# HSarham/automatic-ar

Measured on AMD Instinct MI355X. Metric: LM iterations/sec, higher is better.
Workload: dtype f64

## Files before the change

### automatic-ar_amd/csrc/ba_capi.hip

```cpp
#include <hip/hip_runtime.h>
#include <dlfcn.h>
#include <execinfo.h>
#include <fcntl.h>
#include <unistd.h>
#include <signal.h>

#include <algorithm>
#include <array>
#include <atomic>
#include <chrono>
#include <cmath>
#include <cstring>
#include <map>
#include <numeric>
#include <condition_variable>
#include <mutex>
#include <vector>

#include "../host/internal.h"
#include "../host/se3.h"
#include "geom.hpp"
#include "hostcopy.h"
#include "kernels.h"

// ... 1446 lines not shown
        P.Ad = ((int)dense_ent.size() + 31) / 32 * 32;
        dense_ent.resize(P.Ad, -1);
        const int nga = P.Ad / 16, ngb = P.Ad / 32;
        std::vector<std::vector<uint8_t>> pa(nga, std::vector<uint8_t>(F, 0)), pb(ngb, std::vector<uint8_t>(F, 0));
        for (int f = 0; f < F; f++) {
            pa[0][f] = pb[0][f] = 1;
            for (int s = fslot_start[f]; s < fslot_start[f + 1]; s++) {
                const int dd = dense_of[fslot_ent[s]];
                pa[dd / 16][f] = 1;
                pb[dd / 32][f] = 1;
            }
        }
        struct Blk { int ga, gb; std::vector<int32_t> fr; };
        std::vector<Blk> blks;
        int64_t total_steps = 0;
        for (int ga = 0; ga < nga; ga++)
            for (int gb = 0; gb <= (16 * ga + 15) / 32; gb++) {
                Blk bk{ga, gb, {}};
                for (int f = 0; f < F; f++)
                    if (pa[ga][f] && pb[gb][f]) bk.fr.push_back(f);
                if (bk.fr.empty()) continue;
                total_steps += ((int64_t)bk.fr.size() + 1) / 2;
                blks.push_back(std::move(bk));
            }
        int target = 12 * (int)blks.size();
        if (const char *e = getenv("AAR_SCHUR_SPLIT")) target = std::max(1, atoi(e)) * (int)blks.size();
        const int64_t plen = std::max<int64_t>(16, ((2 * total_steps + target - 1) / target + 3) / 4 * 4);
        struct Piece { int blk; int64_t b, e; int f0; };
        std::vector<Piece> pieces;
        for (size_t k = 0; k < blks.size(); k++)
            for (int64_t b0 = 0; b0 < (int64_t)blks[k].fr.size(); b0 += plen)
                pieces.push_back({(int)k, b0, std::min<int64_t>(b0 + plen, (int64_t)blks[k].fr.size()), blks[k].fr[b0]});
        std::stable_sort(pieces.begin(), pieces.end(), [](const Piece &x, const Piece &y) { return x.f0 < y.f0; });
        for (const Piece &pc : pieces) {
            sm_ga.push_back(blks[pc.blk].ga); sm_gb.push_back(blks[pc.blk].gb);
            sm_fb.push_back((int32_t)sm_frames.size());
            sm_frames.insert(sm_frames.end(), blks[pc.blk].fr.begin() + pc.b, blks[pc.blk].fr.begin() + pc.e);
            sm_fe.push_back((int32_t)sm_frames.size());
        }
        slot_frame.resize(P.total_slots);
        slot_dense.resize(P.total_slots);
        for (int f = 0; f < F; f++)
            for (int s = fslot_start[f]; s < fslot_start[f + 1]; s++) {
                slot_frame[s] = f;
                slot_dense[s] = dense_of[fslot_ent[s]];
            }
        P.n_smwork = (int)sm_ga.size();
    }

    std::vector<int32_t> ent_fixed(A, 0);
    for (int c = 0; c < C; c++) ent_fixed[c] = (c == L.rc || !L.oc) ? 1 : 0;
    for (int m = 0; m < M; m++) ent_fixed[C + m] = (m == L.rm || !L.om) ? 1 : 0;
    for (int e = 0; e < C + M; e++) ent_fixed[e] |= held[e];
    std::vector<double> Kh(d->cam_mats, d->cam_mats + 9 * (size_t)C);

#define UP(field, vec) if ((rc = dev_upload(pb, &P.field, vec))) return fail(rc)
    UP(K, Kh); UP(a_idx, a_idx); UP(a_uv, a_uv); UP(frame_obs_start, frame_obs_start); UP(frame_stride, frame_stride);
    UP(fslot_start, fslot_start); UP(fslot_ent, fslot_ent); UP(b_idx, b_idx); UP(b_uv, b_uv);
    UP(chunk_start, chunk_start); UP(ent_fixed, ent_fixed); UP(up_start, up_start); UP(up_ent, up_ent);
    UP(sw_ent, sw_ent); UP(sw_begin, sw_begin); UP(sw_end, sw_end); UP(pair_rec, pair_rec);
    if (P.use_pcg) {
        const int cus = P.n_cus;
        int64_t longest = 0;
        for (int a = 0; a < A; a++) longest = std::max<int64_t>(longest, pair_base[a + 1] - pair_base[a]);
        int64_t chunk = std::max<int64_t>(256, (total_pairs + 2LL * cus - 1) / (2LL * cus));
        chunk = std::max<int64_t>(chunk, (longest + 7) / 8);
        if (const char *t = getenv("AAR_PCG_CHUNK")) chunk = std::max<int64_t>((longest + 7) / 8, atoll(t));
        std::vector<int32_t> it_ent, it_begin, it_end, ent_item_start(A + 1, 0);
        for (int a = 0; a < A; a++) {
            ent_item_start[a] = (int32_t)it_ent.size();
            const int64_t b0 = pair_base[a], e0 = ent_fixed[a] ? pair_base[a] : pair_base[a + 1];
            int64_t b = b0;
            do {
                const int64_t e = std::min<int64_t>(e0, b + chunk);
                it_ent.push_back(a); it_begin.push_back((int32_t)b); it_end.push_back((int32_t)e);
                b = e;
            } while (b < e0);
        }
        ent_item_start[A] = (int32_t)it_ent.size();
        P.pcg_n_items = (int)it_ent.size();
        UP(pcg_it_ent, it_ent); UP(pcg_it_begin, it_begin); UP(pcg_it_end, it_end); UP(pcg_ent_item_start, ent_item_start);
    }
    if (P.deterministic) { UP(sp_off, sp_off); UP(se_start, se_start); UP(se_items, se_items); UP(pbr_start, pbr_start); UP(pbr_chunk, pbr_chunk); UP(pbr_kind, pbr_kind); UP(pbr_a, pbr_a); UP(pbr_b, pbr_b); }
    if (P.n_smwork) { UP(sm_ga, sm_ga); UP(sm_gb, sm_gb); UP(sm_fb, sm_fb); UP(sm_fe, sm_fe); UP(slot_dense, slot_dense); UP(slot_frame, slot_frame); UP(dense_ent, dense_ent); UP(sm_frames, sm_frames); }
#undef UP
#define AL(field, count) if ((rc = dev_alloc(pb, &P.field, (size_t)(count)))) return fail(rc)
    AL(z[0], 6 * (size_t)(A + F)); AL(z[1], 6 * (size_t)(A + F));
    AL(ent[0], (size_t)(A + F) * ENT_STRIDE); AL(ent[1], (size_t)(A + F) * ENT_STRIDE);
    for (int w = 0; w < 2; w++) {
        AL(blk[w].V, (size_t)F * 36); AL(blk[w].gf, (size_t)F * 6); AL(blk[w].W, (size_t)P.total_slots * 36);
        AL(blk[w].Vinv, (size_t)F * 36); AL(blk[w].hf, (size_t)F * 6);
        AL(blk[w].S, (size_t)P.n_pad * P.n_pad + 2 * (size_t)P.n_pad + 8);
        P.blk[w].rhs = P.blk[w].S + (size_t)P.n_pad * P.n_pad;
        P.blk[w].g0 = P.blk[w].rhs + P.n_pad;
        P.blk[w].tail = P.blk[w].g0 + P.n_pad;
        if (hipMemset(P.blk[w].tail, 0, 8 * sizeof(double)) != hipSuccess) return fail(set_error(AAR_ERR_HIP, "hipMemset failed"));
    }
    if (P.deterministic) { AL(sp_part, (size_t)sp_total); AL(pb_part, (size_t)P.n_chunks * P.pb_stride); }
    if (P.use_pcg) {
        AL(pcg_ws, (size_t)P.pcg_n_items * 28 + 6 * (size_t)F + 8); AL(pcg_counter, 8);
        AL(pcg_yg, (size_t)3 * PCG_NYV * P.n_pad + (size_t)28 * A + 160 + 8); AL(pcg_hop, 2 * PCG_HOP_WORDS);
        if (const char *t = getenv("AAR_PCG_FUSED")) P.pcg_fused = atoi(t) != 0 ? 1 : 0;
        {
            int w32 = 1;
            if (const char *t = getenv("AAR_PCG_W32")) w32 = atoi(t) != 0 ? 1 : 0;
            if (w32 && P.pcg_fused && !P.deterministic && P.pcg_eta >= PCG_W32_MIN_ETA)
// ... 2037 lines not shown
```

### automatic-ar_amd/csrc/kernels.h

```cpp
#pragma once
#include <hip/hip_runtime.h>
#include <stdint.h>
#include <utility>

namespace aar {

constexpr int CHOL_NB = 96;
constexpr int PASSB_CHUNK = 1024;
constexpr int SPCG_MAX_IT = 128, SPCG_BUFS = SPCG_MAX_IT + 2, SPCG_MAX_NT = 14;
inline int spcg_default_cap(int nT) { return nT <= 4 ? 64 : SPCG_MAX_IT; }
constexpr int PCG_NY = 16;
constexpr int PCG_NYV = 2;
constexpr int PCG_HOP_WORDS = (2 * PCG_NY + 1) * 16;
constexpr double PCG_W32_MIN_ETA = 1e-4;
constexpr double SPCG_ABS_TOL_DEFAULT = 2e-5, PCG_ABS_TOL_DEFAULT = 5e-5;
constexpr double SPCG_ETA_DEFAULT = 3e-4, SPCG_ETA_LOOSE_DEFAULT = 0.0, PCG_ETA_DEFAULT = 5e-3, PCG_ETA_LOOSE_DEFAULT = 0.0;
inline int spcg_stride(int n_pad) { return 8 * (n_pad / 6); }


#ifndef SPCG_PRE
#define SPCG_PRE 0
#endif

enum KernelId { KID_UNPACK = 0, KID_RESIDUAL, KID_PASSA, KID_PASSB, KID_MAXDIAG, KID_FRAME_INV, KID_SCHUR, KID_LDL_DIAG,
                KID_LDL_TRSM, KID_LDL_UPDATE, KID_LDL_BACKSOLVE, KID_BACKSUB, KID_REDUCE, KID_LDL_PANEL, KID_PCG, KID_SPCG, KID_SPCG_PRE, KID_PRIOR, KID_COUNT };

struct LaunchHook {
    void (*pre)(void *ctx, int kid) = nullptr;
    void (*post)(void *ctx, int kid) = nullptr;
    void *ctx = nullptr;
};

struct ObsIdx {
    int32_t frame, cam, marker, slots;
};

struct DeviceProblem {
    int C = 0, M = 0, A = 0;
    int intr = 0;
    int F = 0;
    int64_t N = 0;
    int n = 0, n_pad = 0, nT = 0;
    int total_slots = 0, max_kf = 0;
    int n_chunks = 0, n_swork = 0;
    int res_f32 = 1;
    float huber = -1.f;
    double half_size = 0;
    double *K = nullptr;
    ObsIdx *a_idx = nullptr;
    float *a_uv = nullptr;
    int32_t *frame_obs_start = nullptr;
    int32_t *frame_stride = nullptr;
    int32_t *fslot_start = nullptr;
    int32_t *fslot_ent = nullptr;
    ObsIdx *b_idx = nullptr;
    float *b_uv = nullptr;
    int32_t *chunk_start = nullptr;
    int32_t *ent_fixed = nullptr;
    int frames_fixed = 0;
    int32_t *sw_ent = nullptr, *sw_begin = nullptr, *sw_end = nullptr;
    int4 *pair_rec = nullptr;
    int n_smwork = 0;
    int32_t *sm_ga = nullptr, *sm_gb = nullptr, *sm_fb = nullptr, *sm_fe = nullptr, *sm_frames = nullptr;
    int Ad = 0;
    int32_t *slot_dense = nullptr;
    int32_t *slot_frame = nullptr;
    int32_t *dense_ent = nullptr;
    double *Wd = nullptr, *Yd = nullptr;
    int dense_from_passA = 1;
    int deterministic = 0;
    double *pb_part = nullptr;
    int pb_stride = 0, n_pbr = 0;
    int32_t *pbr_start = nullptr, *pbr_chunk = nullptr, *pbr_kind = nullptr, *pbr_a = nullptr, *pbr_b = nullptr;
    double *sp_part = nullptr;
    int64_t *sp_off = nullptr;
    int32_t *se_start = nullptr, *se_items = nullptr;
    int use_pcg = 0, pcg_grid = 0, pcg_max_it = 200;
    double pcg_eta = 0.1;
    double pcg_eta_loose = 0.0, pcg_eta_switch = 0.01, pcg_eta_now = 0.1;
    double pcg_abs_tol = SPCG_ABS_TOL_DEFAULT;
    int pcg_n_items = 0;
    int32_t *pcg_it_ent = nullptr, *pcg_it_begin = nullptr, *pcg_it_end = nullptr, *pcg_ent_item_start = nullptr;
    double *pcg_ws = nullptr;
    int32_t *pcg_counter = nullptr;
    mutable int pcg_parity = 0;
    int n_cus = 256;
    mutable int want_w64 = 0;
    int pcg_fused = 1;
    int pcg_rank0 = 1;
    int pcg_resident = 1;
    int pcg_e_every = 1;
    mutable int pcg_e_age = 0;
    int pcg_coarse = 1, pcg_coarse_from = 8;
    int32_t *up_start = nullptr, *up_ent = nullptr;
    double *pcg_yg = nullptr;
    int32_t *pcg_hop = nullptr;
    int use_spcg = 0, spcg_max_it = 64;
    int spcg_spread = 8;
    int spcg_coarse = 1;
    int spcg_coarse_from = 12;
    mutable int spcg_coarse_on = 0;
    double *spcg_pre = nullptr;
    mutable int spcg_pre_epoch = 0;
    int spcg_root_c = -1, spcg_root_m = -1, spcg_n_free = 0;
    int spcg_test_drop = -1;
    double *spcg_ws = nullptr;
    int32_t *spcg_iters = nullptr;
    mutable int spcg_parity = 0;
    int32_t *spcg_done = nullptr;
    mutable int spcg_epoch = 0;
    double *pcgd_setup = nullptr, *pcgd_minv = nullptr, *pcgd_state = nullptr, *pcgd_y = nullptr, *pcgd_host = nullptr;
    struct Tuning {
        int fused_panel = 3;
        int bs_rides = 1;
        int backsub_rides = 0;
        int lookahead = 1;
        int passA_variant = 0;
        int passAB_occ2 = -1;
        int spcg_backsub_rides = 0;
        int passA_wrench = 1;
        int passB_wrench_merged = 0;
        int passB_lean = 0;
        int pack_system = -1;
        int init_headstart = 1;
    } tune;
    double *z[2] = {nullptr, nullptr};
    double *ent[2] = {nullptr, nullptr};
    struct Blocks {
        double *V = nullptr, *gf = nullptr;
        double *W = nullptr;
        float *Wf = nullptr;
        double *Vinv = nullptr, *hf = nullptr;
        double *S = nullptr;
        double *rhs = nullptr;
        double *g0 = nullptr;
        double *tail = nullptr;
    } blk[2];
    double *Dfac = nullptr;
    double *Linv16 = nullptr;
    double *Lp = nullptr;
    double *zf = nullptr;
    double *delta_s = nullptr;
    int32_t *bs_flags = nullptr;
    mutable int bs_epoch = 0;
    double *err_part = nullptr;
    double *lin_part = nullptr;
    double *scal = nullptr;
    double *host_result = nullptr;
    int32_t *flags = nullptr;
    double *r_out = nullptr;
    int n_prior = 0, prior_rank0 = 1;
    int32_t *prior_ent = nullptr;
    double *prior_dat = nullptr;
    double *prior_out = nullptr;
    LaunchHook hook;
};

void raise_dynamic_lds(const void *kernel, size_t bytes);
template <typename... Params, typename... Args>
inline void launch_lds(void (*kernel)(Params...), dim3 grid, dim3 block, size_t lds, hipStream_t st, Args &&...args) {
    raise_dynamic_lds(reinterpret_cast<const void *>(kernel), lds);
    hipLaunchKernelGGL(kernel, grid, block, lds, st, std::forward<Args>(args)...);
}

struct KTable { const double *base; int stride; };
constexpr int ENT_STRIDE_H = 24;
inline KTable k_table(const DeviceProblem &P, int which) {
    if (P.intr) return KTable{P.ent[which] + (size_t)(P.C + P.M) * ENT_STRIDE_H, ENT_STRIDE_H};
    return KTable{P.K, 9};
}
constexpr int SLOT_C_BITS = 10, SLOT_M_BITS = 11;
inline int pack_slots(int sc, int sm, int sk) { return sc | (sm << SLOT_C_BITS) | (sk << (SLOT_C_BITS + SLOT_M_BITS)); }

extern volatile int g_last_kernel_id;
struct HookScope {
    const DeviceProblem &P;
    int kid;
    HookScope(const DeviceProblem &p, int k) : P(p), kid(k) { g_last_kernel_id = k; if (P.hook.pre) P.hook.pre(P.hook.ctx, kid); }
    ~HookScope() { if (P.hook.post) P.hook.post(P.hook.ctx, kid); }
};

void launch_unpack(const DeviceProblem &P, int which, hipStream_t st, int zero_blk = -1);
void launch_residual(const DeviceProblem &P, int which, double *r_out, hipStream_t st);
void launch_passA(const DeviceProblem &P, int which, double mu_pred, int zero_blk, hipStream_t st);
void launch_passB(const DeviceProblem &P, int which, hipStream_t st);
bool launch_passAB(const DeviceProblem &P, int which, double mu_pred, int zero_blk, hipStream_t st);
size_t passA_lds_bytes(int max_kf, int block);
size_t passA_wrench_lds_bytes(int max_kf, bool intr);
void launch_maxdiag(const DeviceProblem &P, int which, hipStream_t st);
void launch_frame_inv(const DeviceProblem &P, int which, double mu, hipStream_t st, const double *mu_dev = nullptr, double mu_scale = 0.0);
bool launch_schur(const DeviceProblem &P, int which, double sign, hipStream_t st, unsigned long long ride_seq = 0, int ride_n_err = 0,
                  double *ride_scal = nullptr, bool panels_ready = false);
bool launch_chol(const DeviceProblem &P, int which, double mu, hipStream_t st, int trial = -1);
void launch_backsub(const DeviceProblem &P, int cur, int trial, hipStream_t st);
void launch_pcg(const DeviceProblem &P, int which, double mu, hipStream_t st);
size_t pcg_lds_bytes(int A, bool coarse = false);
int pcg_max_grid(int A, bool coarse, int cus);
bool launch_spcg(const DeviceProblem &P, int which, double mu, hipStream_t st, int trial = -1);
int spcg_resident_per_cu(int nT, bool coarse);
inline bool spcg_coarse_now(const DeviceProblem &P) { return P.spcg_coarse && (P.spcg_root_c >= 0 || P.spcg_root_m >= 0); }
bool spcg_fits(int nT);
size_t spcg_ws_doubles(int n_pad);
size_t spcg_pre_doubles(int n_pad);
void spcg_ws_reset(const DeviceProblem &P, hipStream_t st);
void launch_pcgd_setup(const DeviceProblem &P, int which, double mu, hipStream_t st);
void launch_pcgd_iter(const DeviceProblem &P, int which, double mu, int k, bool last, unsigned long long publish_seq, hipStream_t st);
double *pcgd_y_of_launch(const DeviceProblem &P, int k);
void launch_reduce_scalars(const DeviceProblem &P, int n_err, bool fold_shared, unsigned long long publish_seq, hipStream_t st,
                           double *scal_out = nullptr, int maxdiag_blk = -1);
void launch_publish(const DeviceProblem &P, unsigned long long publish_seq, hipStream_t st, const double *src = nullptr, bool flags_reduced = false);
int residual_blocks(const DeviceProblem &P);
constexpr int PRIOR_DAT = 42;
void launch_prior(const DeviceProblem &P, int which, bool add, hipStream_t st);
inline int n_err_terms(const DeviceProblem &P) { return P.F + ((P.n_prior > 0 && P.prior_rank0) ? 1 : 0); }
void launch_track(const DeviceProblem &P, int which, int max_iters, double min_error, double min_step, double min_avg, double tau,
                  int32_t *iters_out, double *err_out, hipStream_t st);

constexpr int SMOOTH_TAIL = 256;
struct SmoothWork {
    double *z[2] = {nullptr, nullptr};
    double *delta = nullptr;
    double *Dg = nullptr, *Of = nullptr;
    double *rhs = nullptr;
    double *Dw = nullptr, *Uw = nullptr, *bw = nullptr, *Dinv = nullptr, *Ls = nullptr;
    double *Ef[2] = {nullptr, nullptr}, *Pe[2] = {nullptr, nullptr};
    double *lin = nullptr;
    double *lam = nullptr;
    double *rel_buf = nullptr;
    const double *rel = nullptr;
    double *res = nullptr;
    int32_t *flag = nullptr;
};
size_t smooth_work_doubles(int F);
void smooth_work_carve(SmoothWork &w, double *base, int F);
void launch_smooth_eval(const DeviceProblem &P, int which, const SmoothWork &w, int cur, bool with_j, hipStream_t st);
int launch_smooth_solve(const SmoothWork &w, int F, double mu, hipStream_t st);

constexpr int LIVE_MAX_W = 16;
constexpr int LIVE_HDR_BYTES = 64;
constexpr int LIVE_REC_BYTES = 48;
constexpr int LIVE_RES_DOUBLES = 24;
constexpr int LIVE_INFO_DOUBLES = 16;
inline size_t live_slot_bytes(int max_obs) {
    return (LIVE_HDR_BYTES + (size_t)(LIVE_REC_BYTES + sizeof(int32_t)) * (size_t)max_obs + 15) / 16 * 16;
}
struct LiveArgs {
    const double *ent, *Kmat;
    const char *ring;
    size_t slot_bytes;
    double *zslot;
    double *anchor;
    double *Ef, *Pe;
    double *res;
// ... 121 lines not shown
```

### automatic-ar_amd/csrc/spcg_kernels.hip

```cpp
#include "geom.hpp"
#include "kernels.h"
#include "backsub.hpp"
#include "wave.hpp"

namespace aar {

namespace {

constexpr unsigned long long SPCG_EMPTY = 0xFFF85EEDFFF85EEDull;

__device__ __forceinline__ bool sp_empty(double v) { return (unsigned long long)__double_as_longlong(v) == SPCG_EMPTY; }
__device__ __forceinline__ void sp_st(double *p, double v) { __hip_atomic_store(p, v, __ATOMIC_RELAXED, __HIP_MEMORY_SCOPE_AGENT); }
__device__ __forceinline__ void sp_st_xcd(double *p, double v) { __hip_atomic_store(p, v, __ATOMIC_RELAXED, __HIP_MEMORY_SCOPE_WORKGROUP); }
__device__ __forceinline__ double sp_ld(const double *p) { return __hip_atomic_load(p, __ATOMIC_RELAXED, __HIP_MEMORY_SCOPE_AGENT); }

__device__ __forceinline__ double rl(double v, int l) {
    return __hiloint2double(__builtin_amdgcn_readlane(__double2hiint(v), l), __builtin_amdgcn_readlane(__double2loint(v), l));
}

}

#ifdef AAR_STAMPS
__device__ unsigned long long g_sp_stamps[512];
__device__ int g_sp_polls[80];
#define SP_STAMP(k) do { __builtin_amdgcn_sched_barrier(0); if (e == e0 && lane == 0 && (k) < 512) g_sp_stamps[k] = __builtin_amdgcn_s_memtime(); __builtin_amdgcn_sched_barrier(0); } while (0)
#define SP_VAL(k, v) do { if (e == e0 && lane == 0 && (k) < 512) g_sp_stamps[k] = (unsigned long long)__double_as_longlong(v); } while (0)
#else
#define SP_STAMP(k) do { } while (0)
#define SP_VAL(k, v) do { } while (0)
#endif

struct SpcgArgs {
    const double *S, *rhs, *g0;
    const int32_t *ent_fixed;
    int n, n_pad;
    double mu, eta2;
    double abs2_mu;
    int max_it;
    double *ws;
    long long set_len;
    int stride, parity;
    double *x_out;
    int32_t *iters;
    int32_t *flags;
    int spread;
    int ride, n_ent_total, n_riders;
    BacksubArgs bs;
    int32_t *done;
    int done_epoch;
    int test_drop;
    const double *pre_rows, *pre_minv, *pre_z, *pre_azt, *pre_share;
    int root_c, root_m;
    int C, M;
};

typedef unsigned int sp_u32x4 __attribute__((ext_vector_type(4)));

template <int NT, bool CO>
__global__ void __launch_bounds__(64) k_spcg(const SpcgArgs a) {
    constexpr int NPAD = 96 * NT, NK = 6 * NT, NENT = 16 * NT, NL = NT, NEB = (NENT + 63) / 64;
    __shared__ __align__(16) double mv[NPAD];
    if (blockIdx.x % a.spread || (int)blockIdx.x >= a.n_ent_total * a.spread) {
        if (!a.ride || blockIdx.x % 8 == 0) return;
        __shared__ double red[32];
        const int bx = (int)blockIdx.x, cg_range = a.n_ent_total * a.spread;
        const int rid = bx < cg_range ? bx - bx / a.spread - 1 : a.n_ent_total * (a.spread - 1) + (bx - cg_range) - (bx - cg_range + 7) / 8;
        for (int blk = rid; blk <= a.bs.n_frame_blocks; blk += a.n_riders) backsub_body(a.bs, blk, red, a.done + 1, a.done_epoch, a.flags);
        return;
    }
    const int lane = threadIdx.x, e = blockIdx.x / a.spread, i = lane >> 3, g = lane & 7;
    auto leave = [&]() {
        if (!a.ride) return;
        asm volatile("s_waitcnt vmcnt(0)" ::: "memory");
        if (lane == 0) {
            const int old = __hip_atomic_fetch_add(a.done, 1, __ATOMIC_RELAXED, __HIP_MEMORY_SCOPE_AGENT);
            if (old + 1 == a.done_epoch * a.n_ent_total) __hip_atomic_store(a.done + 1, a.done_epoch, __ATOMIC_RELAXED, __HIP_MEMORY_SCOPE_AGENT);
        }
    };
    const int n_free_ent = a.n / 6;
    auto fixed = [&](int ent) -> bool { return ent >= n_free_ent || (a.ent_fixed[ent < n_free_ent ? ent : 0] != 0 && !(CO && (ent == a.root_c || ent == a.root_m))); };
    double *set = a.ws + (size_t)a.parity * a.set_len, *other = a.ws + (size_t)(1 - a.parity) * a.set_len;
    const int nprev_raw = a.iters[0];
    {
        const int nprev = min(nprev_raw + 2, SPCG_BUFS);
        for (int bq = lane >> 3; bq < nprev; bq += 8) sp_st(other + (size_t)bq * a.stride + 8 * e + (lane & 7), __longlong_as_double((long long)SPCG_EMPTY));
    }
    if (fixed(e)) {
        if (lane < 6) sp_st(a.x_out + 6 * e + lane, 0.0);
        leave();
        return;
    }
    if (e == a.test_drop) return;
    int e0 = -1, n_act = 0;
#pragma unroll
    for (int k = 0; k < NEB; k++) {
        const unsigned long long fr = __ballot(lane + 64 * k < NENT && !fixed(lane + 64 * k));
        if (e0 < 0 && fr) e0 = 64 * k + __builtin_ctzll(fr);
        n_act += __builtin_popcountll(fr);
    }
    const double xcc = (double)(__builtin_amdgcn_s_getreg(20 | (0 << 6) | (3 << 11)) & 0xf);
    bool same_xcd = false;
    unsigned pact = 0;
#pragma unroll
    for (int k = 0; k < NL; k++) if (!fixed((lane + 64 * k) >> 2)) pact |= 1u << k;
    const bool ra = i < 6;
    const int row = 6 * e + (ra ? i : 0);
    double A2[2 * NK];
    double blk[6][6];
    double r, mi[6], zo[6];
    const bool pseudo = CO && (e == a.root_c || e == a.root_m);
    const int my_root = e < a.C ? a.root_c : (e < a.C + a.M ? a.root_m : -1);
    if (CO) {
        const double *rp = pseudo ? a.pre_azt + (size_t)((e == a.root_c ? 0 : 6) + (ra ? i : 0)) * a.n_pad : a.pre_rows + (size_t)row * a.n_pad;
#pragma unroll
        for (int k = 0; k < NK; k++) {
            const double2 t = reinterpret_cast<const double2 *>(rp)[8 * k + g];
            A2[2 * k] = ra ? t.x : 0.0; A2[2 * k + 1] = ra ? t.y : 0.0;
        }
#pragma unroll
        for (int k = 0; k < 3; k++) {
            const double2 t = reinterpret_cast<const double2 *>(a.pre_minv + 36 * e + 6 * (ra ? i : 0))[k];
            mi[2 * k] = (ra && !pseudo) ? t.x : 0.0; mi[2 * k + 1] = (ra && !pseudo) ? t.y : 0.0;
            const double2 z2 = reinterpret_cast<const double2 *>(a.pre_z + 36 * e + 6 * (ra ? i : 0))[k];
            const bool zon = ra && !pseudo && my_root >= 0;
            zo[2 * k] = zon ? z2.x : 0.0; zo[2 * k + 1] = zon ? z2.y : 0.0;
        }
        r = (ra && !pseudo) ? a.rhs[row] + a.g0[row] : 0.0;
    } else {
        unsigned long long cfx[(NK + 63) / 64] = {};
#pragma unroll
        for (int k = 0; k < NK; k++) {
            const int c0 = 16 * k + 2 * g, c1 = c0 + 1;
            A2[2 * k] = a.S[(c0 <= row) ? (size_t)row * a.n_pad + c0 : (size_t)c0 * a.n_pad + row];
            A2[2 * k + 1] = a.S[(c1 <= row) ? (size_t)row * a.n_pad + c1 : (size_t)c1 * a.n_pad + row];
            if (fixed(c0 / 6)) cfx[k >> 6] |= 1ull << (k & 63);
        }
#pragma unroll
        for (int p = 0; p < 6; p++)
#pragma unroll
            for (int q = 0; q <= p; q++) blk[p][q] = a.S[(size_t)(6 * e + p) * a.n_pad + 6 * e + q];
        r = a.rhs[row] + a.g0[row];
#pragma unroll
        for (int k = 0; k < NK; k++) {
            const int c0 = 16 * k + 2 * g;
            const bool off = !ra || ((cfx[k >> 6] >> (k & 63)) & 1);
            A2[2 * k] = off ? 0.0 : A2[2 * k] + (c0 == row ? a.mu : 0.0);
            A2[2 * k + 1] = off ? 0.0 : A2[2 * k + 1] + (c0 + 1 == row ? a.mu : 0.0);
        }
        if (!ra) r = 0.0;
    }
    SP_STAMP(0);
    SP_STAMP(1);
    if (!CO) {
        double inv[36];
#pragma unroll
        for (int p = 0; p < 6; p++) {
            blk[p][p] += a.mu;
#pragma unroll
            for (int q = 0; q < p; q++) blk[q][p] = blk[p][q];
        }
        if (!spd6_inverse(blk, inv) && lane == 0) atomicOr(a.flags, 2);
#pragma unroll
        for (int k = 0; k < 6; k++) {
            double v = 0.0;
#pragma unroll
            for (int p = 0; p < 6; p++) v = (i == p) ? inv[p * 6 + k] : v;
            mi[k] = v;
        }
    }
    double ec[12];
#pragma unroll
    for (int q = 0; q < 12; q++) ec[q] = 0.0;
    if (CO && pseudo) {
        const int Gq = e == a.root_c ? 0 : 1, elo = Gq ? a.C : 0, ehi = Gq ? a.C + a.M : a.C;
        const int ecl = lane & 7, sg = lane >> 3;
        double acc[10];
#pragma unroll
        for (int t = 0; t < 10; t++) acc[t] = 0.0;
        for (int q0 = elo; q0 < ehi; q0 += 40) {
            double2 v[5][5];
#pragma unroll
            for (int kk = 0; kk < 5; kk++) {
                const int q = q0 + 8 * kk + ecl;
#pragma unroll
                for (int t = 0; t < 5; t++) v[kk][t] = q < ehi ? reinterpret_cast<const double2 *>(a.pre_share + 80 * q + 10 * sg)[t] : make_double2(0.0, 0.0);
            }
#pragma unroll
            for (int kk = 0; kk < 5; kk++)
#pragma unroll
                for (int t = 0; t < 5; t++) { acc[2 * t] += v[kk][t].x; acc[2 * t + 1] += v[kk][t].y; }
        }
#pragma unroll
        for (int t = 0; t < 10; t++) acc[t] = sum8(acc[t]);
        if (ecl == 0) {
#pragma unroll
            for (int t = 0; t < 5; t++) reinterpret_cast<double2 *>(mv + 10 * sg)[t] = make_double2(acc[2 * t], acc[2 * t + 1]);
        }
        __builtin_amdgcn_wave_barrier();
        double eb[6][6], inv[36];
#pragma unroll
        for (int p = 0; p < 6; p++)
#pragma unroll
            for (int q = 0; q <= p; q++) { const double v = mv[12 * p + 6 * Gq + q]; eb[p][q] = v; eb[q][p] = v; }
        if (!spd6_inverse(eb, inv) && lane == 0) atomicOr(a.flags, 2);
#pragma unroll
        for (int k = 0; k < 6; k++) {
            double v = 0.0;
#pragma unroll
            for (int p = 0; p < 6; p++) v = (i == p) ? inv[p * 6 + k] : v;
            mi[k] = v;
        }
#pragma unroll
        for (int b = 0; b < 12; b++) ec[b] = ra ? mv[12 * i + b] : 0.0;
        r = ra ? mv[72 + i] : 0.0;
        __builtin_amdgcn_wave_barrier();
    }
    auto prec = [&](double w) -> double {
        double s = 0.0;
#pragma unroll
        for (int k = 0; k < 6; k++) s = fma(mi[k], rl(w, 8 * k), s);
        return s;
    };
    bool dead = false;
    auto publish = [&](int b, double val, double s1, double s2) {
        double *rec = set + (size_t)b * a.stride + 8 * e;
        double sh = (g & 1) ? s1 : s2;
        sh += dpp<DPP_ROR8>(sh);
        sh = sum_across_rows(sh);
        const bool is_m = ra && g == 0, is_s = lane == 1 || lane == 2;
        if (is_m || is_s) {
            if (same_xcd) sp_st_xcd(rec + (is_m ? i : 5 + lane), is_m ? val : sh);
            else sp_st(rec + (is_m ? i : 5 + lane), is_m ? val : sh);
        }
    };
    const __amdgpu_buffer_rsrc_t rsrc = __builtin_amdgcn_make_buffer_rsrc(set, 0, (int)(a.set_len * 8), 0x00020000);
    auto gather = [&](int b, double &t1, double &t2) {
        const int soff = b * a.stride * 8;
        double2 cur[NL];
#pragma unroll
        for (int k = 0; k < NL; k++) cur[k] = ((pact >> k) & 1) ? make_double2(__longlong_as_double((long long)SPCG_EMPTY), __longlong_as_double((long long)SPCG_EMPTY)) : make_double2(0.0, 0.0);
        long spins = 0;
        if (SPCG_PRE > 0) __builtin_amdgcn_s_sleep(SPCG_PRE);
        for (;;) {
            sp_u32x4 t[NL];
#pragma unroll
            for (int k = 0; k < NL; k++)
                if (sp_empty(cur[k].x) || sp_empty(cur[k].y)) t[k] = __builtin_amdgcn_raw_buffer_load_b128(rsrc, 16 * (lane + 64 * k), soff, 16 );
            bool ok = true;
#pragma unroll
            for (int k = 0; k < NL; k++) {
                if (sp_empty(cur[k].x) || sp_empty(cur[k].y)) {
                    const double lo = __hiloint2double((int)t[k][1], (int)t[k][0]), hi = __hiloint2double((int)t[k][3], (int)t[k][2]);
                    if (sp_empty(cur[k].x)) cur[k].x = lo;
                    if (sp_empty(cur[k].y)) cur[k].y = hi;
                    ok = ok && !sp_empty(cur[k].x) && !sp_empty(cur[k].y);
                }
            }
            if (__ballot(!ok) == 0ull) break;
#ifdef AAR_STAMPS
            if (e == e0 && lane == 0 && b < 80) g_sp_polls[b]++;
#endif
            if (++spins > (1L << 19)) { dead = true; break; }
            __builtin_amdgcn_s_sleep(1);
        }
        SP_STAMP(300 + b);
        const int w2 = lane & 3;
        double sg = 0.0, sd = 0.0;
#pragma unroll
        for (int k = 0; k < NL; k++) {
// ... 214 lines not shown
    if (tid < 72) {
        const int i = tid / 12, c = tid % 12;
        const double v = (az[tid] + az[72 + tid]) + az[144 + tid];
        az[tid] = v;
        a.azt[(size_t)c * a.n_pad + 6 * j + i] = v;
        const int root = c < 6 ? a.root_c : a.root_m;
        if (root >= 0) al[i * a.n_pad + 6 * root + (c % 6)] = v;
    }
    __syncthreads();
    for (int q = tid; q < 3 * a.n_pad; q += 256) reinterpret_cast<double2 *>(a.rows + (size_t)6 * j * a.n_pad)[q] = reinterpret_cast<const double2 *>(al)[q];
    const double *Zj = zl + 36 * j;
    if (tid < 36) a.z[36 * j + tid] = Zj[tid];
    if (pose && tid >= 64 && tid < 64 + 78) {
        const int o = tid - 64;
        double v = 0.0;
        if (o < 72) {
            const int c = o / 12, b = o % 12;
#pragma unroll
            for (int i = 0; i < 6; i++) v = fma(Zj[6 * i + c], az[12 * i + b], v);
        } else {
#pragma unroll
            for (int i = 0; i < 6; i++) v = fma(Zj[6 * i + (o - 72)], bj[i], v);
        }
        a.share[80 * j + o] = v;
    }
}

size_t spcg_pre_lds_bytes(int n_pad) { return sizeof(double) * ((size_t)36 * (n_pad / 6) + (size_t)6 * n_pad + 224) + sizeof(int32_t) * (n_pad / 6 + 2); }
size_t spcg_pre_doubles(int n_pad) { const size_t ne = n_pad / 6; return (size_t)n_pad * n_pad + 36 * ne + 36 * ne + (size_t)12 * n_pad + 80 * ne + 8; }

static void launch_spcg_pre(const DeviceProblem &P, int which, double mu, hipStream_t st, SpcgArgs &k) {
    const size_t ne = P.n_pad / 6;
    SpcgPreArgs a;
    a.S = P.blk[which].S; a.rhs = P.blk[which].rhs; a.g0 = P.blk[which].g0; a.ent = P.ent[which]; a.ent_fixed = P.ent_fixed;
    a.n = P.n; a.n_pad = P.n_pad; a.n_ent = (int)ne; a.C = P.C; a.M = P.M; a.mu = mu;
    a.root_c = P.spcg_root_c; a.root_m = P.spcg_root_m;
    double *w = P.spcg_pre;
    a.rows = w; w += (size_t)P.n_pad * P.n_pad;
    a.minv = w; w += 36 * ne;
    a.z = w; w += 36 * ne;
    a.azt = w; w += (size_t)12 * P.n_pad;
    a.share = w; w += 80 * ne;
    a.flags = P.flags;
    k.pre_rows = a.rows; k.pre_minv = a.minv; k.pre_z = a.z; k.pre_azt = a.azt; k.pre_share = a.share; k.root_c = a.root_c; k.root_m = a.root_m;
    HookScope _h(P, KID_SPCG_PRE);
    launch_lds(k_spcg_pre, dim3((unsigned)ne), dim3(256), spcg_pre_lds_bytes(P.n_pad), st, a);
}

bool spcg_fits(int nT) { return nT >= 1 && nT <= SPCG_MAX_NT; }
int spcg_resident_per_cu(int nT, bool coarse) {
    int nb = 0;
    hipError_t rc = hipErrorInvalidValue;
    switch (nT) {
#define SPCG_CASE(t) case t: { int nc = 1 << 30; if (coarse) rc = hipOccupancyMaxActiveBlocksPerMultiprocessor(&nc, k_spcg<t, true>, 64, 0); \
                               if (!coarse || rc == hipSuccess) rc = hipOccupancyMaxActiveBlocksPerMultiprocessor(&nb, k_spcg<t, false>, 64, 0); nb = std::min(nb, nc); } break;
        SPCG_CASE(1) SPCG_CASE(2) SPCG_CASE(3) SPCG_CASE(4) SPCG_CASE(5) SPCG_CASE(6) SPCG_CASE(7) SPCG_CASE(8)
        SPCG_CASE(9) SPCG_CASE(10) SPCG_CASE(11) SPCG_CASE(12) SPCG_CASE(13) SPCG_CASE(14)
#undef SPCG_CASE
        default: break;
    }
    if (rc != hipSuccess) { (void)hipGetLastError(); return 0; }
    return nb;
}
size_t spcg_ws_doubles(int n_pad) { return (size_t)2 * SPCG_BUFS * spcg_stride(n_pad); }
void spcg_ws_reset(const DeviceProblem &P, hipStream_t st) {
    (void)hipMemsetD32Async(reinterpret_cast<hipDeviceptr_t>(P.spcg_ws), (int)0xFFF85EED, 2 * spcg_ws_doubles(P.n_pad), st);
    (void)hipMemsetAsync(P.spcg_done, 0, 2 * sizeof(int32_t), st);
    P.spcg_epoch = 0;
}

bool launch_spcg(const DeviceProblem &P, int which, double mu, hipStream_t st, int trial) {
    const DeviceProblem::Blocks &b = P.blk[which];
    SpcgArgs a;
    a.S = b.S; a.rhs = b.rhs; a.g0 = b.g0; a.ent_fixed = P.ent_fixed; a.n = P.n; a.n_pad = P.n_pad;
    a.mu = mu; a.eta2 = P.pcg_eta_now * P.pcg_eta_now; a.abs2_mu = P.pcg_abs_tol * P.pcg_abs_tol * mu; a.max_it = std::min(P.spcg_max_it, SPCG_MAX_IT);
    a.ws = P.spcg_ws; a.stride = spcg_stride(P.n_pad); a.set_len = (long long)SPCG_BUFS * a.stride; a.parity = P.spcg_parity;
    a.x_out = P.delta_s; a.iters = P.spcg_iters; a.flags = P.flags; a.test_drop = P.spcg_test_drop;
    a.pre_rows = a.pre_minv = a.pre_z = a.pre_azt = a.pre_share = nullptr; a.root_c = a.root_m = -1; a.C = P.C; a.M = P.M;
    const bool coarse = spcg_coarse_now(P) && P.spcg_coarse_on;
    if (coarse) launch_spcg_pre(P, which, mu, st, a);
    a.spread = P.spcg_spread;
    P.spcg_parity ^= 1;
    const int n_ent = P.n_pad / 6;
    a.n_ent_total = n_ent;
    a.ride = (trial >= 0 && P.tune.spcg_backsub_rides && a.spread >= 8 && !P.hook.pre && P.F > 0) ? 1 : 0;
    a.bs = backsub_args(P, which, trial >= 0 ? trial : which, 1);
    a.done = P.spcg_done; a.done_epoch = 0; a.n_riders = 0;
    int grid = n_ent * a.spread;
    if (a.ride) {
        a.done_epoch = ++P.spcg_epoch;
        const int base = n_ent * (a.spread - 1), want = std::min(a.bs.n_frame_blocks + 1, 4096);
        int extra = 0;
        if (base < want) extra = ((want - base) * 8 + 6) / 7;
        grid += extra;
        a.n_riders = base + extra - (extra + 7) / 8;
    }
    HookScope _h(P, KID_SPCG);
    switch (P.nT) {
#define SPCG_CASE(t) case t: if (coarse) hipLaunchKernelGGL((k_spcg<t, true>), dim3(grid), dim3(64), 0, st, a); \
                             else hipLaunchKernelGGL((k_spcg<t, false>), dim3(grid), dim3(64), 0, st, a); break;
        SPCG_CASE(1) SPCG_CASE(2) SPCG_CASE(3) SPCG_CASE(4) SPCG_CASE(5) SPCG_CASE(6) SPCG_CASE(7) SPCG_CASE(8)
        SPCG_CASE(9) SPCG_CASE(10) SPCG_CASE(11) SPCG_CASE(12) SPCG_CASE(13) SPCG_CASE(14)
#undef SPCG_CASE
        default: break;
    }
    return a.ride != 0;
}

}
```

Measured before the change: 13370.

## Stage SPCG Schur slab through LDS, pass fixed mask by value, split rider kernel

```diff
diff --git a/automatic-ar_amd/csrc/ba_capi.hip b/automatic-ar_amd/csrc/ba_capi.hip
--- a/automatic-ar_amd/csrc/ba_capi.hip
+++ b/automatic-ar_amd/csrc/ba_capi.hip
@@ -1522,6 +1522,7 @@
     for (int c = 0; c < C; c++) ent_fixed[c] = (c == L.rc || !L.oc) ? 1 : 0;
     for (int m = 0; m < M; m++) ent_fixed[C + m] = (m == L.rm || !L.om) ? 1 : 0;
     for (int e = 0; e < C + M; e++) ent_fixed[e] |= held[e];
+    spcg_build_fixed_mask(P, ent_fixed.data());
     std::vector<double> Kh(d->cam_mats, d->cam_mats + 9 * (size_t)C);
 
 #define UP(field, vec) if ((rc = dev_upload(pb, &P.field, vec))) return fail(rc)
diff --git a/automatic-ar_amd/csrc/kernels.h b/automatic-ar_amd/csrc/kernels.h
--- a/automatic-ar_amd/csrc/kernels.h
+++ b/automatic-ar_amd/csrc/kernels.h
@@ -8,6 +8,9 @@
 constexpr int CHOL_NB = 96;
 constexpr int PASSB_CHUNK = 1024;
 constexpr int SPCG_MAX_IT = 128, SPCG_BUFS = SPCG_MAX_IT + 2, SPCG_MAX_NT = 14;
+constexpr int SPCG_MASK_WORDS = (16 * SPCG_MAX_NT + 63) / 64;
+constexpr int SPCG_STAGE_MAX_NT = 5;
+constexpr int SPCG_RIDE_MAX_NT = 8;
 inline int spcg_default_cap(int nT) { return nT <= 4 ? 64 : SPCG_MAX_IT; }
 constexpr int PCG_NY = 16;
 constexpr int PCG_NYV = 2;
@@ -103,6 +106,7 @@
     double *spcg_pre = nullptr;
     mutable int spcg_pre_epoch = 0;
     int spcg_root_c = -1, spcg_root_m = -1, spcg_n_free = 0;
+    unsigned long long spcg_fixed[SPCG_MASK_WORDS] = {~0ull, ~0ull, ~0ull, ~0ull};
     int spcg_test_drop = -1;
     double *spcg_ws = nullptr;
     int32_t *spcg_iters = nullptr;
@@ -199,6 +203,7 @@
 bool launch_spcg(const DeviceProblem &P, int which, double mu, hipStream_t st, int trial = -1);
 int spcg_resident_per_cu(int nT, bool coarse);
 inline bool spcg_coarse_now(const DeviceProblem &P) { return P.spcg_coarse && (P.spcg_root_c >= 0 || P.spcg_root_m >= 0); }
+void spcg_build_fixed_mask(DeviceProblem &P, const int32_t *ent_fixed_host);
 bool spcg_fits(int nT);
 size_t spcg_ws_doubles(int n_pad);
 size_t spcg_pre_doubles(int n_pad);
diff --git a/automatic-ar_amd/csrc/spcg_kernels.hip b/automatic-ar_amd/csrc/spcg_kernels.hip
--- a/automatic-ar_amd/csrc/spcg_kernels.hip
+++ b/automatic-ar_amd/csrc/spcg_kernels.hip
@@ -1,3 +1,4 @@
+#include <type_traits>
 #include "geom.hpp"
 #include "kernels.h"
 #include "backsub.hpp"
@@ -25,15 +26,21 @@
 __device__ int g_sp_polls[80];
 #define SP_STAMP(k) do { __builtin_amdgcn_sched_barrier(0); if (e == e0 && lane == 0 && (k) < 512) g_sp_stamps[k] = __builtin_amdgcn_s_memtime(); __builtin_amdgcn_sched_barrier(0); } while (0)
 #define SP_VAL(k, v) do { if (e == e0 && lane == 0 && (k) < 512) g_sp_stamps[k] = (unsigned long long)__double_as_longlong(v); } while (0)
+#define SP_ENTRY() unsigned long long sp_t_entry; do { __builtin_amdgcn_sched_barrier(0); sp_t_entry = __builtin_amdgcn_s_memtime(); __builtin_amdgcn_sched_barrier(0); } while (0)
+#define SP_ENTRY_PUT(k) do { if (e == e0 && lane == 0) g_sp_stamps[k] = sp_t_entry; } while (0)
+#define SP_DRAIN() asm volatile("s_waitcnt vmcnt(0) lgkmcnt(0)" ::: "memory")
 #else
 #define SP_STAMP(k) do { } while (0)
 #define SP_VAL(k, v) do { } while (0)
+#define SP_ENTRY() do { } while (0)
+#define SP_ENTRY_PUT(k) do { } while (0)
+#define SP_DRAIN() do { } while (0)
 #endif
 
 struct SpcgArgs {
     const double *S, *rhs, *g0;
-    const int32_t *ent_fixed;
-    int n, n_pad;
+    unsigned long long fixed_mask[SPCG_MASK_WORDS];
+    int n_pad;
     double mu, eta2;
     double abs2_mu;
     int max_it;
@@ -44,57 +51,70 @@
     int32_t *iters;
     int32_t *flags;
     int spread;
-    int ride, n_ent_total, n_riders;
-    BacksubArgs bs;
-    int32_t *done;
-    int done_epoch;
     int test_drop;
     const double *pre_rows, *pre_minv, *pre_z, *pre_azt, *pre_share;
     int root_c, root_m;
     int C, M;
 };
+struct SpcgRideArgs : SpcgArgs {
+    int n_riders;
+    BacksubArgs bs;
+    int32_t *done;
+    int done_epoch;
+};
 
 typedef unsigned int sp_u32x4 __attribute__((ext_vector_type(4)));
 
-template <int NT, bool CO>
-__global__ void __launch_bounds__(64) k_spcg(const SpcgArgs a) {
+template <int NT, bool CO, bool RIDE>
+__global__ void __launch_bounds__(64) k_spcg(const std::conditional_t<RIDE, SpcgRideArgs, SpcgArgs> a) {
     constexpr int NPAD = 96 * NT, NK = 6 * NT, NENT = 16 * NT, NL = NT, NEB = (NENT + 63) / 64;
-    __shared__ __align__(16) double mv[NPAD];
-    if (blockIdx.x % a.spread || (int)blockIdx.x >= a.n_ent_total * a.spread) {
-        if (!a.ride || blockIdx.x % 8 == 0) return;
-        __shared__ double red[32];
-        const int bx = (int)blockIdx.x, cg_range = a.n_ent_total * a.spread;
-        const int rid = bx < cg_range ? bx - bx / a.spread - 1 : a.n_ent_total * (a.spread - 1) + (bx - cg_range) - (bx - cg_range + 7) / 8;
-        for (int blk = rid; blk <= a.bs.n_frame_blocks; blk += a.n_riders) backsub_body(a.bs, blk, red, a.done + 1, a.done_epoch, a.flags);
+    constexpr bool STAGED = !CO && NT <= SPCG_STAGE_MAX_NT;
+    __shared__ __align__(16) double lds[STAGED ? 6 * NPAD : NPAD];
+    double *const mv = lds;
+    if (blockIdx.x % a.spread || (int)blockIdx.x >= NENT * a.spread) {
+        if constexpr (RIDE) {
+            if (blockIdx.x % 8 == 0) return;
+            __shared__ double red[32];
+            const int bx = (int)blockIdx.x, cg_range = NENT * a.spread;
+            const int rid = bx < cg_range ? bx - bx / a.spread - 1 : NENT * (a.spread - 1) + (bx - cg_range) - (bx - cg_range + 7) / 8;
+            for (int blk = rid; blk <= a.bs.n_frame_blocks; blk += a.n_riders) backsub_body(a.bs, blk, red, a.done + 1, a.done_epoch, a.flags);
+        }
         return;
     }
     const int lane = threadIdx.x, e = blockIdx.x / a.spread, i = lane >> 3, g = lane & 7;
+    SP_ENTRY();
     auto leave = [&]() {
-        if (!a.ride) return;
-        asm volatile("s_waitcnt vmcnt(0)" ::: "memory");
-        if (lane == 0) {
-            const int old = __hip_atomic_fetch_add(a.done, 1, __ATOMIC_RELAXED, __HIP_MEMORY_SCOPE_AGENT);
-            if (old + 1 == a.done_epoch * a.n_ent_total) __hip_atomic_store(a.done + 1, a.done_epoch, __ATOMIC_RELAXED, __HIP_MEMORY_SCOPE_AGENT);
+        if constexpr (RIDE) {
+            asm volatile("s_waitcnt vmcnt(0)" ::: "memory");
+            if (lane == 0) {
+                const int old = __hip_atomic_fetch_add(a.done, 1, __ATOMIC_RELAXED, __HIP_MEMORY_SCOPE_AGENT);
+                if (old + 1 == a.done_epoch * NENT) __hip_atomic_store(a.done + 1, a.done_epoch, __ATOMIC_RELAXED, __HIP_MEMORY_SCOPE_AGENT);
+            }
         }
     };
-    const int n_free_ent = a.n / 6;
-    auto fixed = [&](int ent) -> bool { return ent >= n_free_ent || (a.ent_fixed[ent < n_free_ent ? ent : 0] != 0 && !(CO && (ent == a.root_c || ent == a.root_m))); };
+    auto fixed = [&](int ent) -> bool {
+        unsigned long long w = a.fixed_mask[0];
+#pragma unroll
+        for (int q = 1; q < NEB; q++) w = (ent >> 6) == q ? a.fixed_mask[q] : w;
+        return ((w >> (ent & 63)) & 1ull) != 0ull;
+    };
     double *set = a.ws + (size_t)a.parity * a.set_len, *other = a.ws + (size_t)(1 - a.parity) * a.set_len;
     const int nprev_raw = a.iters[0];
-    {
+    auto clear_other = [&]() {
         const int nprev = min(nprev_raw + 2, SPCG_BUFS);
         for (int bq = lane >> 3; bq < nprev; bq += 8) sp_st(other + (size_t)bq * a.stride + 8 * e + (lane & 7), __longlong_as_double((long long)SPCG_EMPTY));
-    }
+    };
     if (fixed(e)) {
+        clear_other();
         if (lane < 6) sp_st(a.x_out + 6 * e + lane, 0.0);
         leave();
         return;
     }
-    if (e == a.test_drop) return;
+    if (e == a.test_drop) { clear_other(); return; }
     int e0 = -1, n_act = 0;
 #pragma unroll
     for (int k = 0; k < NEB; k++) {
-        const unsigned long long fr = __ballot(lane + 64 * k < NENT && !fixed(lane + 64 * k));
+        const unsigned long long fr = ~a.fixed_mask[k] & (NENT - 64 * k >= 64 ? ~0ull : (1ull << ((NENT - 64 * k) & 63)) - 1ull);
         if (e0 < 0 && fr) e0 = 64 * k + __builtin_ctzll(fr);
         n_act += __builtin_popcountll(fr);
     }
@@ -125,21 +145,79 @@
             const bool zon = ra && !pseudo && my_root >= 0;
             zo[2 * k] = zon ? z2.x : 0.0; zo[2 * k + 1] = zon ? z2.y : 0.0;
         }
-        r = (ra && !pseudo) ? a.rhs[row] + a.g0[row] : 0.0;
+        const double r_b = a.rhs[row], r_g = a.g0[row];
+        clear_other();
+        SP_ENTRY_PUT(440); SP_STAMP(441); SP_DRAIN(); SP_STAMP(442);
+        r = (ra && !pseudo) ? r_b + r_g : 0.0;
     } else {
         unsigned long long cfx[(NK + 63) / 64] = {};
 #pragma unroll
-        for (int k = 0; k < NK; k++) {
-            const int c0 = 16 * k + 2 * g, c1 = c0 + 1;
-            A2[2 * k] = a.S[(c0 <= row) ? (size_t)row * a.n_pad + c0 : (size_t)c0 * a.n_pad + row];
-            A2[2 * k + 1] = a.S[(c1 <= row) ? (size_t)row * a.n_pad + c1 : (size_t)c1 * a.n_pad + row];
-            if (fixed(c0 / 6)) cfx[k >> 6] |= 1ull << (k & 63);
-        }
-#pragma unroll
-        for (int p = 0; p < 6; p++)
-#pragma unroll
-            for (int q = 0; q <= p; q++) blk[p][q] = a.S[(size_t)(6 * e + p) * a.n_pad + 6 * e + q];
-        r = a.rhs[row] + a.g0[row];
+        for (int k = 0; k < NK; k++) if (fixed((16 * k + 2 * g) / 6)) cfx[k >> 6] |= 1ull << (k & 63);
+        double r_b, r_g;
+        if constexpr (STAGED) {
+            constexpr int NRP = (3 * NPAD + 63) / 64, NCP = (3 * (NPAD - 6) + 63) / 64;
+            const double2 *slab = reinterpret_cast<const double2 *>(a.S + (size_t)6 * e * NPAD);
+            const double2 *below = reinterpret_cast<const double2 *>(a.S + (size_t)(6 * e + 6) * NPAD + 6 * e);
+            const int wcol = 3 * e + 3;
+            double2 rp[NRP], cp[NCP];
+#pragma unroll
+            for (int j = 0; j < NRP; j++) {
+                const int c = lane + 64 * j;
+                rp[j] = (c < 3 * NPAD && c % (NPAD / 2) < wcol) ? slab[c] : make_double2(0.0, 0.0);
+            }
+#pragma unroll
+            for (int j = 0; j < NCP; j++) {
+                const int c = lane + 64 * j, rr = c / 3, t = c - 3 * rr;
+                cp[j] = (6 * e + 6 + rr < NPAD) ? below[(size_t)rr * (NPAD / 2) + t] : make_double2(0.0, 0.0);
+            }
+            r_b = a.rhs[row]; r_g = a.g0[row];
+            clear_other();
+            SP_ENTRY_PUT(440); SP_STAMP(441); SP_DRAIN(); SP_STAMP(442);
+#pragma unroll
+            for (int j = 0; j < NRP; j++) {
+                const int c = lane + 64 * j;
+                if (c < 3 * NPAD && c % (NPAD / 2) < wcol) reinterpret_cast<double2 *>(lds)[c] = rp[j];
+            }
+#pragma unroll
+            for (int j = 0; j < NCP; j++) {
+                const int c = lane + 64 * j, rr = c / 3, t = c - 3 * rr, rw = 6 * e + 6 + rr;
+                if (rw < NPAD) { lds[(2 * t) * NPAD + rw] = cp[j].x; lds[(2 * t + 1) * NPAD + rw] = cp[j].y; }
+            }
+            __builtin_amdgcn_wave_barrier();
+            {
+                const int p = lane / 6, q = lane - 6 * p;
+                const bool up = lane < 36 && q > p;
+                const double v = up ? lds[q * NPAD + 6 * e + p] : 0.0;
+                __builtin_amdgcn_wave_barrier();
+                if (up) lds[p * NPAD + 6 * e + q] = v;
+                __builtin_amdgcn_wave_barrier();
+            }
+#pragma unroll
+            for (int k = 0; k < NK; k++) {
+                const double2 t = reinterpret_cast<const double2 *>(lds + (ra ? i : 0) * NPAD)[8 * k + g];
+                A2[2 * k] = t.x; A2[2 * k + 1] = t.y;
+            }
+#pragma unroll
+            for (int p = 0; p < 6; p++)
+#pragma unroll
+                for (int q = 0; q <= p; q++) blk[p][q] = lds[p * NPAD + 6 * e + q];
+            __builtin_amdgcn_wave_barrier();
+        } else {
+#pragma unroll
+            for (int k = 0; k < NK; k++) {
+                const int c0 = 16 * k + 2 * g, c1 = c0 + 1;
+                A2[2 * k] = a.S[(c0 <= row) ? row * NPAD + c0 : c0 * NPAD + row];
+                A2[2 * k + 1] = a.S[(c1 <= row) ? row * NPAD + c1 : c1 * NPAD + row];
+            }
+#pragma unroll
+            for (int p = 0; p < 6; p++)
+#pragma unroll
+                for (int q = 0; q <= p; q++) blk[p][q] = a.S[(6 * e + p) * NPAD + 6 * e + q];
+            r_b = a.rhs[row]; r_g = a.g0[row];
+            clear_other();
+            SP_ENTRY_PUT(440); SP_STAMP(441); SP_DRAIN(); SP_STAMP(442);
+        }
+        r = r_b + r_g;
 #pragma unroll
         for (int k = 0; k < NK; k++) {
             const int c0 = 16 * k + 2 * g;
@@ -215,6 +293,7 @@
         r = ra ? mv[72 + i] : 0.0;
         __builtin_amdgcn_wave_barrier();
     }
+    SP_STAMP(443);
     auto prec = [&](double w) -> double {
         double s = 0.0;
 #pragma unroll
@@ -535,8 +614,8 @@
     int nb = 0;
     hipError_t rc = hipErrorInvalidValue;
     switch (nT) {
-#define SPCG_CASE(t) case t: { int nc = 1 << 30; if (coarse) rc = hipOccupancyMaxActiveBlocksPerMultiprocessor(&nc, k_spcg<t, true>, 64, 0); \
-                               if (!coarse || rc == hipSuccess) rc = hipOccupancyMaxActiveBlocksPerMultiprocessor(&nb, k_spcg<t, false>, 64, 0); nb = std::min(nb, nc); } break;
+#define SPCG_CASE(t) case t: { int nc = 1 << 30; if (coarse) rc = hipOccupancyMaxActiveBlocksPerMultiprocessor(&nc, k_spcg<t, true, false>, 64, 0); \
+                               if (!coarse || rc == hipSuccess) rc = hipOccupancyMaxActiveBlocksPerMultiprocessor(&nb, k_spcg<t, false, false>, 64, 0); nb = std::min(nb, nc); } break;
         SPCG_CASE(1) SPCG_CASE(2) SPCG_CASE(3) SPCG_CASE(4) SPCG_CASE(5) SPCG_CASE(6) SPCG_CASE(7) SPCG_CASE(8)
         SPCG_CASE(9) SPCG_CASE(10) SPCG_CASE(11) SPCG_CASE(12) SPCG_CASE(13) SPCG_CASE(14)
 #undef SPCG_CASE
@@ -555,39 +634,59 @@
 bool launch_spcg(const DeviceProblem &P, int which, double mu, hipStream_t st, int trial) {
     const DeviceProblem::Blocks &b = P.blk[which];
     SpcgArgs a;
-    a.S = b.S; a.rhs = b.rhs; a.g0 = b.g0; a.ent_fixed = P.ent_fixed; a.n = P.n; a.n_pad = P.n_pad;
+    a.S = b.S; a.rhs = b.rhs; a.g0 = b.g0; a.n_pad = P.n_pad;
+    for (int q = 0; q < SPCG_MASK_WORDS; q++) a.fixed_mask[q] = P.spcg_fixed[q];
     a.mu = mu; a.eta2 = P.pcg_eta_now * P.pcg_eta_now; a.abs2_mu = P.pcg_abs_tol * P.pcg_abs_tol * mu; a.max_it = std::min(P.spcg_max_it, SPCG_MAX_IT);
     a.ws = P.spcg_ws; a.stride = spcg_stride(P.n_pad); a.set_len = (long long)SPCG_BUFS * a.stride; a.parity = P.spcg_parity;
     a.x_out = P.delta_s; a.iters = P.spcg_iters; a.flags = P.flags; a.test_drop = P.spcg_test_drop;
     a.pre_rows = a.pre_minv = a.pre_z = a.pre_azt = a.pre_share = nullptr; a.root_c = a.root_m = -1; a.C = P.C; a.M = P.M;
     const bool coarse = spcg_coarse_now(P) && P.spcg_coarse_on;
-    if (coarse) launch_spcg_pre(P, which, mu, st, a);
+    if (coarse) {
+        launch_spcg_pre(P, which, mu, st, a);
+        for (int root : {a.root_c, a.root_m})
+            if (root >= 0) a.fixed_mask[root >> 6] &= ~(1ull << (root & 63));
+    }
     a.spread = P.spcg_spread;
     P.spcg_parity ^= 1;
     const int n_ent = P.n_pad / 6;
-    a.n_ent_total = n_ent;
-    a.ride = (trial >= 0 && P.tune.spcg_backsub_rides && a.spread >= 8 && !P.hook.pre && P.F > 0) ? 1 : 0;
-    a.bs = backsub_args(P, which, trial >= 0 ? trial : which, 1);
-    a.done = P.spcg_done; a.done_epoch = 0; a.n_riders = 0;
-    int grid = n_ent * a.spread;
-    if (a.ride) {
-        a.done_epoch = ++P.spcg_epoch;
-        const int base = n_ent * (a.spread - 1), want = std::min(a.bs.n_frame_blocks + 1, 4096);
+    const int grid = n_ent * a.spread;
+    const bool ride = trial >= 0 && P.tune.spcg_backsub_rides && a.spread >= 8 && P.nT <= SPCG_RIDE_MAX_NT && !P.hook.pre && P.F > 0;
+    HookScope _h(P, KID_SPCG);
+    if (ride) {
+        SpcgRideArgs ar;
+        static_cast<SpcgArgs &>(ar) = a;
+        ar.bs = backsub_args(P, which, trial, 1);
+        ar.done = P.spcg_done; ar.done_epoch = ++P.spcg_epoch;
+        const int base = n_ent * (a.spread - 1), want = std::min(ar.bs.n_frame_blocks + 1, 4096);
         int extra = 0;
         if (base < want) extra = ((want - base) * 8 + 6) / 7;
-        grid += extra;
-        a.n_riders = base + extra - (extra + 7) / 8;
-    }
-    HookScope _h(P, KID_SPCG);
+        ar.n_riders = base + extra - (extra + 7) / 8;
+        switch (P.nT) {
+#define SPCG_CASE(t) case t: if (coarse) hipLaunchKernelGGL((k_spcg<t, true, true>), dim3(grid + extra), dim3(64), 0, st, ar); \
+                             else hipLaunchKernelGGL((k_spcg<t, false, true>), dim3(grid + extra), dim3(64), 0, st, ar); break;
+            SPCG_CASE(1) SPCG_CASE(2) SPCG_CASE(3) SPCG_CASE(4) SPCG_CASE(5) SPCG_CASE(6) SPCG_CASE(7) SPCG_CASE(8)
+#undef SPCG_CASE
+            default: break;
+        }
+        static_assert(SPCG_RIDE_MAX_NT == 8, "one riding instantiation per tile count that can ride");
+        return true;
+    }
     switch (P.nT) {
-#define SPCG_CASE(t) case t: if (coarse) hipLaunchKernelGGL((k_spcg<t, true>), dim3(grid), dim3(64), 0, st, a); \
-                             else hipLaunchKernelGGL((k_spcg<t, false>), dim3(grid), dim3(64), 0, st, a); break;
+#define SPCG_CASE(t) case t: if (coarse) hipLaunchKernelGGL((k_spcg<t, true, false>), dim3(grid), dim3(64), 0, st, a); \
+                             else hipLaunchKernelGGL((k_spcg<t, false, false>), dim3(grid), dim3(64), 0, st, a); break;
         SPCG_CASE(1) SPCG_CASE(2) SPCG_CASE(3) SPCG_CASE(4) SPCG_CASE(5) SPCG_CASE(6) SPCG_CASE(7) SPCG_CASE(8)
         SPCG_CASE(9) SPCG_CASE(10) SPCG_CASE(11) SPCG_CASE(12) SPCG_CASE(13) SPCG_CASE(14)
 #undef SPCG_CASE
         default: break;
     }
-    return a.ride != 0;
-}
-
-}
+    return false;
+}
+
+void spcg_build_fixed_mask(DeviceProblem &P, const int32_t *ent_fixed_host) {
+    const int n_free_ent = P.n / 6;
+    for (int q = 0; q < SPCG_MASK_WORDS; q++) P.spcg_fixed[q] = 0ull;
+    for (int ent = 0; ent < 64 * SPCG_MASK_WORDS; ent++)
+        if (ent >= n_free_ent || ent_fixed_host[ent] != 0) P.spcg_fixed[ent >> 6] |= 1ull << (ent & 63);
+}
+
+}
```

New measurement: 14040, median of 6. 1.05x the previous value.
